# pliam1105/BoxFusion

Measured on AMD Instinct MI355X. Metric: RGB-D frames/sec (whole node) on 640x480 stream, higher is better.
Workload: dtype bf16; 1 GPU; configs[2]: synthetic 640x480 RGB-D, batch 8/step/GPU, gap=1, CuTR ViT-B RGB-D + CLIP ViT-H/14 x16 crops/frame + fusion; frames=440, global_batch=8, parallelism=dp1, inflight_batches_per_gpu=2, scene_objects=30, fused_boxes=83, global_boxes=30

## Files before the change

### boxfusion_amd/_lib.py

```python
from __future__ import annotations

import atexit
import ctypes
import threading
import weakref
import sys
import os

import numpy as np
import torch

HERE = os.path.dirname(os.path.abspath(__file__))
LIB_PATH = os.environ.get("BF_LIB_PATH") or os.path.join(HERE, "libboxfusion_hip.so")
_LIB = None

c_int, c_float, c_double, c_void_p, c_size_t = (ctypes.c_int, ctypes.c_float, ctypes.c_double,
                                                ctypes.c_void_p, ctypes.c_size_t)

BF_DEV_FUSION_LIST_OVERFLOW = 1
BF_DEV_HULL_OVERFLOW = 2
BF_DEV_VIEW_OVERFLOW = 4
BF_DEV_INDEX_RANGE = 8
BF_DEV_HULL_TRUNC = 16

# ... 539 lines not shown
    o_bs = sq * o.stride(0) if o_bs is None else o_bs
    if o_map is not None:
        _need(o_map, torch.int32, "o_map")
        if o_map.numel() < batch * sq:
            raise HipError(f"o_map has {o_map.numel()} rows < batch*sq = {batch * sq}")
    LL = ctypes.c_longlong
    _check(lib().bf_attention_bf16_ex(c_void_p(q.data_ptr()), c_void_p(k.data_ptr()),
                                      c_void_p(v.data_ptr()), c_void_p(o.data_ptr()), c_int(batch),
                                      c_int(heads), c_int(sq), c_int(sk), c_int(head_dim),
                                      c_int(q.stride(0)), c_int(k.stride(0)), c_int(v.stride(0)),
                                      c_int(o.stride(0)), LL(q_bs), LL(k_bs), LL(v_bs), LL(o_bs),
                                      c_float(scale), _ptr(o_map) if o_map is not None else None,
                                      c_int(variant or _knobs().get("attn_variant", 0)), _stream()),
           "bf_attention_bf16_ex")
    return o


def attention_fp8out(q, k, v, o, batch, heads, sq, sk, head_dim, scale, out_qscale, q_bs=None,
                     k_bs=None, v_bs=None, o_bs=None, variant=0):
    for x, n in ((q, "q"), (k, "k"), (v, "v")):
        _need(x, torch.bfloat16, n)
    _need(o, FP8, "o")
    q_bs = sq * q.stride(0) if q_bs is None else q_bs
    k_bs = sk * k.stride(0) if k_bs is None else k_bs
    v_bs = sk * v.stride(0) if v_bs is None else v_bs
    o_bs = sq * o.stride(0) if o_bs is None else o_bs
    LL = ctypes.c_longlong
    _check(lib().bf_attention_fp8out_ex(c_void_p(q.data_ptr()), c_void_p(k.data_ptr()), c_void_p(v.data_ptr()),
                                        c_void_p(o.data_ptr()), c_int(batch), c_int(heads), c_int(sq),
                                        c_int(sk), c_int(head_dim), c_int(q.stride(0)), c_int(k.stride(0)),
                                        c_int(v.stride(0)), c_int(o.stride(0)), LL(q_bs), LL(k_bs), LL(v_bs),
                                        LL(o_bs), c_float(scale), c_float(out_qscale),
                                        c_int(variant or _knobs().get("attn_variant", 0)), _stream()),
           "bf_attention_fp8out_ex")
    return o


def layernorm(x, weight, bias, eps, out=None, row_map=None, out_dtype=torch.bfloat16):
    _need(x, torch.float32, "x")
    M, C = x.shape
    if out is None:
        out = torch.empty((M, C), dtype=out_dtype, device=x.device)
    if out.dtype not in (torch.bfloat16, torch.float32) or x.stride(1) != 1 or out.stride(1) != 1:
        raise HipError("layernorm: f32 in, bf16 / f32 out, unit column stride")
    _check(lib().bf_layernorm_out(c_void_p(x.data_ptr()), c_int(x.stride(0)), _ptr(weight),
                                  _ptr(bias), c_float(eps), c_void_p(out.data_ptr()),
                                  c_int(out.stride(0)), c_int(int(out.dtype == torch.float32)),
                                  _ptr(row_map) if row_map is not None else None, c_int(M), c_int(C),
                                  _stream()), "bf_layernorm_out")
    return out



def attention_causal(q, k, v, o, batch, heads, s, head_dim, scale):
    for x, n in ((q, "q"), (k, "k"), (v, "v"), (o, "o")):
        _need(x, torch.bfloat16, n)
    LL = ctypes.c_longlong
    _check(lib().bf_attention_causal(c_void_p(q.data_ptr()), c_void_p(k.data_ptr()), c_void_p(v.data_ptr()),
                                     c_void_p(o.data_ptr()), c_int(batch), c_int(heads), c_int(s),
                                     c_int(head_dim), c_int(q.stride(0)), c_int(k.stride(0)),
                                     c_int(v.stride(0)), c_int(o.stride(0)), LL(s * q.stride(0)),
                                     LL(s * k.stride(0)), LL(s * v.stride(0)), LL(s * o.stride(0)),
                                     c_float(scale), _stream()), "bf_attention_causal")
    return o


def token_embed(ids, table, pos, out=None, status=None):
    _need(ids, torch.int32, "ids")
    _need(table, torch.float32, "table")
    _need(pos, torch.float32, "pos")
    N, S = ids.shape
    W = table.shape[1]
    if pos.shape[0] < S or pos.shape[1] != W:
        raise HipError(f"token_embed: positional table {tuple(pos.shape)} for S={S}, W={W}")
    if out is None:
        out = torch.empty((N * S, W), dtype=torch.float32, device=ids.device)
    _need(out, torch.float32, "out")
    own = status is None
    if own:
        status = torch.zeros(1, dtype=torch.int32, device=ids.device)
    _check(lib().bf_token_embed(_ptr(ids), c_int(N * S), _ptr(table), c_int(table.shape[0]), _ptr(pos),
                                c_int(S), c_int(W), _ptr(out), _ptr(status), _stream()), "bf_token_embed")
    if own and int(status.item()) & BF_DEV_INDEX_RANGE:
        raise HipError("bf_token_embed: a token id outside the vocabulary (BF_DEV_INDEX_RANGE)")
    return out


def text_pool(ids, x, out=None):
    _need(ids, torch.int32, "ids")
    _need(x, torch.float32, "x")
    N, S = ids.shape
    W = x.shape[1]
    if out is None:
        out = torch.empty((N, W), dtype=torch.float32, device=x.device)
    _need(out, torch.float32, "out")
    _check(lib().bf_text_pool(_ptr(ids), c_int(N), c_int(S), _ptr(x), c_int(W), _ptr(out), _stream()),
           "bf_text_pool")
    return out


def l2_normalize_rows(x, out=None):
    _need(x, torch.float32, "x")
    if out is None:
        out = torch.empty_like(x)
    _need(out, torch.float32, "out")
    _check(lib().bf_l2_normalize_rows(_ptr(x), c_int(x.shape[0]), c_int(x.shape[1]), _ptr(out), _stream()),
           "bf_l2_normalize_rows")
    return out


def ingest_rgbd(bgr, depth_u16, depth_scale, rot_k=0, rgb_out=None, depth_out=None, src_bgr=True):
    _need(bgr, torch.uint8, "bgr")
    if bgr.dim() == 3:
        bgr = bgr[None]
    F_, Hc, Wc, C = bgr.shape
    if C != 3:
# ... 722 lines not shown
```

### boxfusion_amd/csrc/bf_attn.hip

```cpp
#include "bf_common.h"

#include <type_traits>
#include <climits>
#include <algorithm>

typedef __bf16 bf16x8 __attribute__((ext_vector_type(8)));
typedef float f32x16 __attribute__((ext_vector_type(16)));
typedef unsigned short u16;

#define AT_THREADS 256
#define AT_QT 128
#define AT_KT 64

struct alignas(16) V128 {
    uint32_t x, y, z, w;
};
struct alignas(8) V64 {
    uint32_t x, y;
};

__device__ __forceinline__ u16 at_f2bf(float f) {
    __bf16 b = (__bf16)f;
    return *reinterpret_cast<u16*>(&b);
}

__device__ __forceinline__ long long attn_out_offset(const int32_t* __restrict__ o_map, int b, int q,
                                                     int sq, long long o_bs, int o_rs) {
    if (!o_map) return b * o_bs + (long long)q * o_rs;
    if (q >= sq) return -1;
    const int r = o_map[(long long)b * sq + q];
    return r < 0 ? -1 : (long long)r * o_rs;
}


typedef short s16x4 __attribute__((ext_vector_type(4)));


struct AttnBlk {
    int qb, h, b;
};
__device__ __forceinline__ AttnBlk attn_block(int remap) {
    const unsigned nx = gridDim.x, ny = gridDim.y, nz = gridDim.z;
    if (!remap) return AttnBlk{(int)blockIdx.x, (int)blockIdx.y, (int)blockIdx.z};
    const unsigned n = nx * ny * nz;
    const unsigned id = blockIdx.x + nx * (blockIdx.y + ny * blockIdx.z);
    const unsigned xcd = id % 8u, k = id / 8u, q = n / 8u, r = n % 8u;
    const unsigned lin = (xcd < r ? xcd * (q + 1) : r * (q + 1) + (xcd - r) * q) + k;
    return AttnBlk{(int)(lin % nx), (int)((lin / nx) % ny), (int)(lin / (nx * ny))};
}

__host__ __device__ constexpr int attn_vrow_bytes(int d) {
    int sb = 2 * d;
    while (sb % 256 != 64 && sb % 256 != 192) sb += 32;
    return sb;
}

#define AT2_THR 8.0f

template <int D, int DB, bool ONES>
__device__ __forceinline__ void attn2_softmax(f32x16 (&s)[2], bool sub1, bool mask, int k0, int sk,
                                              int fh, float c, float& m_run, float& l_run,
                                              f32x16 (&o)[DB], bf16x8 (&pf)[2][2], int kmax = INT_MAX) {
    if (mask) {
        const int klim = min(sk - 1, kmax);
#pragma unroll
        for (int sub = 0; sub < 2; ++sub)
#pragma unroll
            for (int e = 0; e < 16; ++e) {
                const int key = k0 + sub * 32 + (e & 3) + 8 * (e >> 2) + 4 * fh;
                s[sub][e] = (key <= klim) ? s[sub][e] : -INFINITY;
            }
    }
    float mt = s[0][0];
#pragma unroll
    for (int e = 1; e < 16; ++e) mt = fmaxf(mt, s[0][e]);
    if (sub1) {
#pragma unroll
        for (int e = 0; e < 16; ++e) mt = fmaxf(mt, s[1][e]);
    }
    mt = fmaxf(mt, __shfl_xor(mt, 32, 64)) * c;
    if (__any(mt > m_run + AT2_THR)) {
        const float m_new = fmaxf(m_run, mt);
        const float alpha = __builtin_amdgcn_exp2f(m_run - m_new);
        m_run = m_new;
        l_run *= alpha;
#pragma unroll
        for (int db = 0; db < DB; ++db)
#pragma unroll
            for (int e = 0; e < 16; ++e) o[db][e] *= alpha;
    }
    float ls = 0.f;
#pragma unroll
    for (int sub = 0; sub < 2; ++sub) {
        if (sub == 1 && !sub1) {
#pragma unroll
            for (int e = 0; e < 16; ++e) pf[1][e >> 3][e & 7] = (__bf16)0.0f;
            continue;
        }
#pragma unroll
        for (int e = 0; e < 16; ++e) {
            const float p = __builtin_amdgcn_exp2f(fmaf(s[sub][e], c, -m_run));
            if (!ONES) ls += p;
            pf[sub][e >> 3][e & 7] = (__bf16)p;
        }
    }
    if (!ONES) l_run += ls;
}

#ifndef ATTN_WPE64
#define ATTN_WPE64 3
#endif
#ifndef ATTN_WPE80
#define ATTN_WPE80 3
#endif
template <int D, int NW, bool F8O = false, bool CAUSAL = false, bool LSTQ = false>
__global__ void __launch_bounds__(NW * 64, (D == 64 && NW == 4) ? ATTN_WPE64 : (D == 80 && NW == 4 && !CAUSAL) ? ATTN_WPE80 : 1)
k_attn2(const u16* __restrict__ Q, const u16* __restrict__ K,
                                                      const u16* __restrict__ V, u16* __restrict__ O,
                                                      int sq, int sk, int q_rs, int k_rs, int v_rs,
                                                      int o_rs, long long q_bs, long long k_bs,
                                                      long long v_bs, long long o_bs, float scale_log2,
                                                      const int32_t* __restrict__ o_map, float oqs = 1.f) {
    constexpr int KS = D / 16;
    constexpr int DB = (D + 31) / 32;
    constexpr bool ONES = (D % 32) != 0;
    constexpr int KROW = D + 8;
    constexpr int VROW = attn_vrow_bytes(D) / 2;
    constexpr int KTILE = AT_KT * KROW;
    constexpr int VTILE = AT_KT * VROW;
    constexpr int CPR = D / 8;
    constexpr int CH = AT_KT * CPR;
    constexpr int NT = NW * 64;
    constexpr int NBUF = 2;
    __shared__ __attribute__((aligned(16))) u16 sK[NBUF * KTILE];
    __shared__ __attribute__((aligned(16))) u16 sV[NBUF * VTILE];
    constexpr bool LST = LSTQ && !CAUSAL && D % 16 == 0;
    constexpr int EB = F8O ? 1 : 2;
    constexpr int OROW = ((EB * D + 16) / 32) * 32 + 16;
    constexpr bool OWN = NW >= 8;
    static_assert(!LST || OWN || NW * 32 * OROW <= NBUF * KTILE * 2, "staged rows fit the K ring");
    __shared__ __attribute__((aligned(16))) unsigned char sO[LST && OWN ? NW * 32 * OROW : 16];

    const int t = threadIdx.x, lane = t & 63, wave = t >> 6;
    const AttnBlk blk = attn_block(1);
    const int h = blk.h, b = blk.b;
    const int fr = lane & 31, fh = lane >> 5;
    const int q = blk.qb * (NW * 32) + wave * 32 + fr;
    const bool idle = blk.qb * (NW * 32) + wave * 32 >= sq;
    const u16* Qb = Q + b * q_bs + h * D;
    const u16* Kb = K + b * k_bs + h * D;
    const u16* Vb = V + b * v_bs + h * D;

    bf16x8 qf[KS];
#pragma unroll
    for (int ks = 0; ks < KS; ++ks)
        qf[ks] = *reinterpret_cast<const bf16x8*>(Qb + (size_t)min(q, sq - 1) * q_rs + 16 * ks + 8 * fh);
    if (VROW > D)
        for (int i = t; i < NBUF * AT_KT * (VROW - D); i += NT) {
            const int r = i / (VROW - D), c = i % (VROW - D);
            sV[r * VROW + D + c] = (ONES && c == 0) ? (u16)0x3F80 : (u16)0;
        }

    static_assert(CH % 64 == 0 && NT % 64 == 0, "wave-uniform staging guard");
    constexpr int NTS = NT;
    const int ts = t;
    constexpr int NSO = (CH + NTS - 1) / NTS;
    typedef unsigned u32x4 __attribute__((ext_vector_type(4)));
    u32x4 stk[NSO], stv[NSO];
    int srow[NSO], scol[NSO];
#pragma unroll
    for (int i = 0; i < NSO; ++i) {
        const int c = min(ts + i * NTS, CH - 1);
        srow[i] = c / CPR;
        scol[i] = (c % CPR) * 8;
    }
    auto stage_load = [&](int k0_) {
#pragma unroll
        for (int i = 0; i < NSO; ++i) {
            const int key = min(k0_ + srow[i], sk - 1);
            stk[i] = *reinterpret_cast<const u32x4*>(Kb + (size_t)key * k_rs + scol[i]);
            stv[i] = *reinterpret_cast<const u32x4*>(Vb + (size_t)key * v_rs + scol[i]);
        }
    };
    auto stage_store = [&](int buf_) {
#pragma unroll
        for (int i = 0; i < NSO; ++i) {
            if (ts + i * NTS < CH) {
                *reinterpret_cast<u32x4*>(sK + buf_ * KTILE + srow[i] * KROW + scol[i]) = stk[i];
                *reinterpret_cast<u32x4*>(sV + buf_ * VTILE + srow[i] * VROW + scol[i]) = stv[i];
            }
        }
    };

    f32x16 o[DB];
#pragma unroll
    for (int db = 0; db < DB; ++db)
#pragma unroll
        for (int e = 0; e < 16; ++e) o[db][e] = 0.f;
    float m_run = -INFINITY, l_run = 0.f;
    const int g16 = (lane >> 4) & 1, q4 = (lane & 15) >> 2, p4 = lane & 3;
    const int ntiles = (sk + AT_KT - 1) / AT_KT;
    const int nfull = sk / AT_KT;

    auto qk = [&](int tile, f32x16 (&s)[2], bool maybe_tail) {
        const int k0 = tile * AT_KT;
        const u16* kt = sK + (tile % NBUF) * KTILE;
        const bool sub1 = !maybe_tail || (k0 + 32 < sk);
#pragma unroll
        for (int sub = 0; sub < 2; ++sub) {
            if (sub == 1 && !sub1) {
#pragma unroll
                for (int e = 0; e < 16; ++e) s[1][e] = -INFINITY;
                continue;
            }
#pragma unroll
            for (int ks = 0; ks < KS; ++ks) {
                bf16x8 kf = *reinterpret_cast<const bf16x8*>(kt + (sub * 32 + fr) * KROW + 16 * ks + 8 * fh);
                s[sub] = __builtin_amdgcn_mfma_f32_32x32x16_bf16(kf, qf[ks], ks == 0 ? f32x16{} : s[sub], 0, 0, 0);
            }
        }
    };
    auto sm_pv = [&](int tile, f32x16 (&s)[2], auto mask_tag) {
        constexpr bool MASK = decltype(mask_tag)::value;
        const int k0 = tile * AT_KT;
        const u16* kt = sK + (tile % NBUF) * KTILE;
        const u16* vt = sV + (tile % NBUF) * VTILE;
        const bool sub1 = !MASK || (k0 + 32 < sk);
        bf16x8 pf[2][2];
        attn2_softmax<D, DB, ONES>(s, sub1, MASK, k0, sk, fh, scale_log2, m_run, l_run, o, pf,
                                   CAUSAL ? q : INT_MAX);
#pragma unroll
        for (int db = 0; db < DB; ++db) {
            const int d0 = db * 32 + g16 * 16 + 4 * p4;
#pragma unroll
            for (int sub = 0; sub < 2; ++sub)
#pragma unroll
                for (int ss = 0; ss < 2; ++ss) {
                    if (MASK && sub == 1 && !sub1) continue;
                    const int kb = 32 * sub + 16 * ss + 4 * fh + q4;
                    typedef __attribute__((address_space(3))) s16x4* lds_s4;
                    const s16x4 lo = __builtin_amdgcn_ds_read_tr16_b64_v4i16((lds_s4)(vt + kb * VROW + d0));
                    const s16x4 hi = __builtin_amdgcn_ds_read_tr16_b64_v4i16((lds_s4)(vt + (kb + 8) * VROW + d0));
                    typedef short s16x8 __attribute__((ext_vector_type(8)));
                    const s16x8 lohi = __builtin_shufflevector(lo, hi, 0, 1, 2, 3, 4, 5, 6, 7);
                    o[db] = __builtin_amdgcn_mfma_f32_32x32x16_bf16(__builtin_bit_cast(bf16x8, lohi),
                                                                   pf[sub][ss], o[db], 0, 0, 0);
                }
        }
    };
    auto tile_body = [&](int tile, auto mask_tag) {
        f32x16 s[2];
        qk(tile, s, decltype(mask_tag)::value);
        sm_pv(tile, s, mask_tag);
    };

    stage_load(0);
    stage_store(0);
    __syncthreads();
    if constexpr (CAUSAL) {
        const int nt = min(ntiles, (min(blk.qb * (NW * 32) + NW * 32, sq) - 1) / AT_KT + 1);
        for (int tile = 0; tile < nt; ++tile) {
            const bool more = tile + 1 < nt;
            if (more) stage_load((tile + 1) * AT_KT);
            tile_body(tile, std::true_type{});
            if (more) stage_store((tile + 1) & 1);
            __syncthreads();
        }
    } else {
        for (int tile = 0; tile < nfull; ++tile) {
            const bool more = tile + 1 < ntiles;
            if (more) stage_load((tile + 1) * AT_KT);
            if (!idle) tile_body(tile, std::false_type{});
            if (more) stage_store((tile + 1) % NBUF);
            __syncthreads();
        }
        if (nfull < ntiles && !idle) tile_body(nfull, std::true_type{});
    }
    float l;
    if (ONES) {
        constexpr int rr = D % 32;
        constexpr int e_l = ((rr >> 3) << 2) | (rr & 3);
        constexpr int fh_l = (rr >> 2) & 1;
        const float mine = o[DB - 1][e_l];
        const float other = __shfl_xor(mine, 32, 64);
        l = (fh == fh_l) ? mine : other;
    } else {
        l = l_run + __shfl_xor(l_run, 32, 64);
    }
    if constexpr (LST) {
        const float inv = 1.0f / l;
        if constexpr (!OWN) __syncthreads();
        if (idle) return;
        unsigned char* wreg = (OWN ? sO : reinterpret_cast<unsigned char*>(sK)) + wave * 32 * OROW;
#pragma unroll
        for (int db = 0; db < DB; ++db)
#pragma unroll
            for (int g = 0; g < 4; ++g) {
                const int d0 = db * 32 + 8 * g + 4 * fh;
                if (d0 >= D) continue;
                if constexpr (F8O) {
                    const float sc = inv * oqs;
                    float a[4];
#pragma unroll
                    for (int i = 0; i < 4; ++i) a[i] = fminf(fmaxf(o[db][4 * g + i] * sc, -448.f), 448.f);
                    int pk = __builtin_amdgcn_cvt_pk_fp8_f32(a[0], a[1], 0, false);
                    pk = __builtin_amdgcn_cvt_pk_fp8_f32(a[2], a[3], pk, true);
                    *reinterpret_cast<int*>(wreg + fr * OROW + d0) = pk;
                } else {
                    V64 w;
                    w.x = (uint32_t)at_f2bf(o[db][4 * g + 0] * inv) | ((uint32_t)at_f2bf(o[db][4 * g + 1] * inv) << 16);
                    w.y = (uint32_t)at_f2bf(o[db][4 * g + 2] * inv) | ((uint32_t)at_f2bf(o[db][4 * g + 3] * inv) << 16);
                    *reinterpret_cast<V64*>(wreg + fr * OROW + 2 * d0) = w;
                }
            }
        constexpr int CPRO = EB * D / 16;
        unsigned char* Ob = reinterpret_cast<unsigned char*>(O);
#pragma unroll
        for (int j = 0; j < (32 * CPRO + 63) / 64; ++j) {
            const int c = lane + 64 * j;
            if (c >= 32 * CPRO) break;
            const int r = c / CPRO, col = c % CPRO;
            const int qr = q - fr + r;
            const V128 val = *reinterpret_cast<const V128*>(wreg + r * OROW + 16 * col);
            const long long off = attn_out_offset(o_map, b, qr, sq, o_bs, o_rs);
            if (qr < sq && off >= 0) *reinterpret_cast<V128*>(Ob + EB * (off + h * D) + 16 * col) = val;
        }
        return;
    }
    const long long o_off = attn_out_offset(o_map, b, q, sq, o_bs, o_rs);
    if (q < sq && o_off >= 0) {
        const float inv = 1.0f / l;
        if constexpr (F8O) {
            unsigned char* orow = reinterpret_cast<unsigned char*>(O) + o_off + h * D;
            const float sc = inv * oqs;
#pragma unroll
            for (int db = 0; db < DB; ++db)
#pragma unroll
                for (int g = 0; g < 4; ++g) {
                    const int d0 = db * 32 + 8 * g + 4 * fh;
                    if (d0 >= D) continue;
                    float a[4];
#pragma unroll
                    for (int i = 0; i < 4; ++i) a[i] = fminf(fmaxf(o[db][4 * g + i] * sc, -448.f), 448.f);
                    int pk = __builtin_amdgcn_cvt_pk_fp8_f32(a[0], a[1], 0, false);
                    pk = __builtin_amdgcn_cvt_pk_fp8_f32(a[2], a[3], pk, true);
                    *reinterpret_cast<int*>(orow + d0) = pk;
                }
        } else {
            u16* orow = O + o_off + h * D;
#pragma unroll
            for (int db = 0; db < DB; ++db)
#pragma unroll
                for (int g = 0; g < 4; ++g) {
                    const int d0 = db * 32 + 8 * g + 4 * fh;
                    if (d0 >= D) continue;
                    V64 w;
                    w.x = (uint32_t)at_f2bf(o[db][4 * g + 0] * inv) | ((uint32_t)at_f2bf(o[db][4 * g + 1] * inv) << 16);
                    w.y = (uint32_t)at_f2bf(o[db][4 * g + 2] * inv) | ((uint32_t)at_f2bf(o[db][4 * g + 3] * inv) << 16);
                    *reinterpret_cast<V64*>(orow + d0) = w;
                }
        }
    }
}
BF_API int bf_attention_bf16_ex(const void* q, const void* k, const void* v, void* o, int batch,
                                int heads, int sq, int sk, int head_dim, int q_rs, int k_rs,
                                int v_rs, int o_rs, long long q_bs, long long k_bs, long long v_bs,
                                long long o_bs, float scale, const int32_t* o_map, int variant,
                                void* stream) {
    const int av = variant == 0 ? 6 : variant;
    if (!q || !k || !v || !o || batch <= 0 || heads <= 0 || sq <= 0 || sk <= 0) return BF_ERR_ARG;
    if ((q_rs | k_rs | v_rs) % 8 != 0 || o_rs % 4 != 0) return BF_ERR_UNSUPPORTED;
    const float sl2 = scale * 1.4426950408889634f;
    const int nw_one = (sq + 31) / 32;
    const bool short_s = nw_one > 4 && nw_one <= 9;
    const bool lst = av != 27;
    const int mid = av == 28 ? 9 : av == 29 ? 4 : av == 30 ? 8
                  : (head_dim == 64 || head_dim == 80) ? 4 : 8;
    const bool four_all = av == 31;
    const int top = av == 28 ? 9 : (four_all || head_dim == 80) ? 4 : 9;
    const bool eight = short_s && nw_one <= 8 && mid == 8 && !four_all;
    const bool nine = short_s && !four_all && (nw_one <= 8 ? mid == 9 : top == 9);
    const bool wide8 = head_dim == 64 && sq > 448 && sq <= 512 && av != 33;
    const hipStream_t st = bf_stream(stream);
#define LAUNCH_2(DD, NWV, LS)                                                                     \
    hipLaunchKernelGGL((k_attn2<DD, NWV, false, false, LS>), dim3((sq + NWV * 32 - 1) / (NWV * 32), heads, batch), \
                       dim3(NWV * 64), 0, st, (const u16*)q, (const u16*)k, (const u16*)v, (u16*)o, sq, sk, \
                       q_rs, k_rs, v_rs, o_rs, q_bs, k_bs, v_bs, o_bs, sl2, o_map, 1.f)
#define LAUNCH_2D(DD)                                                                             \
    if (nw_one <= 2) { LAUNCH_2(DD, 2, false); }                                                  \
    else if (eight) { if (lst) { LAUNCH_2(DD, 8, true); } else { LAUNCH_2(DD, 8, false); } }      \
    else if (nine) { if (lst) { LAUNCH_2(DD, 9, true); } else { LAUNCH_2(DD, 9, false); } }       \
    else if (wide8) { if (lst) { LAUNCH_2(DD, 8, true); } else { LAUNCH_2(DD, 8, false); } }      \
    else { if (lst) { LAUNCH_2(DD, 4, true); } else { LAUNCH_2(DD, 4, false); } }
    switch (head_dim) {
        case 32: LAUNCH_2D(32); break;
        case 64: LAUNCH_2D(64); break;
        case 80: LAUNCH_2D(80); break;
        case 128: LAUNCH_2(128, 4, false); break;
        default: return BF_ERR_UNSUPPORTED;
    }
#undef LAUNCH_2D
#undef LAUNCH_2
    return bf_check_launch();
}

BF_API int bf_attention_bf16_omap(const void* q, const void* k, const void* v, void* o, int batch,
                                  int heads, int sq, int sk, int head_dim, int q_rs, int k_rs,
                                  int v_rs, int o_rs, long long q_bs, long long k_bs, long long v_bs,
                                  long long o_bs, float scale, const int32_t* o_map, void* stream) {
    return bf_attention_bf16_ex(q, k, v, o, batch, heads, sq, sk, head_dim, q_rs, k_rs, v_rs, o_rs, q_bs, k_bs,
                                v_bs, o_bs, scale, o_map, 0, stream);
}

BF_API int bf_attention_bf16(const void* q, const void* k, const void* v, void* o, int batch,
                             int heads, int sq, int sk, int head_dim, int q_rs, int k_rs, int v_rs,
                             int o_rs, long long q_bs, long long k_bs, long long v_bs,
                             long long o_bs, float scale, void* stream) {
    return bf_attention_bf16_omap(q, k, v, o, batch, heads, sq, sk, head_dim, q_rs, k_rs, v_rs, o_rs,
                                  q_bs, k_bs, v_bs, o_bs, scale, nullptr, stream);
}

BF_API int bf_attention_fp8out_ex(const void* q, const void* k, const void* v, void* o, int batch,
                                  int heads, int sq, int sk, int head_dim, int q_rs, int k_rs, int v_rs,
                                  int o_rs, long long q_bs, long long k_bs, long long v_bs, long long o_bs,
                                  float scale, float out_qscale, int variant, void* stream) {
    const int av = variant == 0 ? 6 : variant;
    if (!q || !k || !v || !o || batch <= 0 || heads <= 0 || sq <= 0 || sk <= 0 || !(out_qscale > 0.f))
        return BF_ERR_ARG;
    if ((q_rs | k_rs | v_rs) % 8 != 0 || o_rs % 4 != 0 || o_bs % 4 != 0) return BF_ERR_UNSUPPORTED;
    const float sl2 = scale * 1.4426950408889634f;
    const int nw_one = (sq + 31) / 32;
    const bool lst = av != 27;
    const hipStream_t st = bf_stream(stream);
#define LAUNCH_8(DD, NWV, LS)                                                                     \
    hipLaunchKernelGGL((k_attn2<DD, NWV, true, false, LS>), dim3((sq + NWV * 32 - 1) / (NWV * 32), heads, batch), \
                       dim3(NWV * 64), 0, st, (const u16*)q, (const u16*)k, (const u16*)v, (u16*)o, sq, sk, \
                       q_rs, k_rs, v_rs, o_rs, q_bs, k_bs, v_bs, o_bs, sl2, (const int32_t*)nullptr, out_qscale)
    const bool nine = nw_one > 4 && nw_one <= 9 && !(head_dim == 80 && nw_one == 9 && av != 28);
#define LAUNCH_8D(DD)                                                                             \
    if (nine) { if (lst) { LAUNCH_8(DD, 9, true); } else { LAUNCH_8(DD, 9, false); } }             \
    else { if (lst) { LAUNCH_8(DD, 4, true); } else { LAUNCH_8(DD, 4, false); } }
    switch (head_dim) {
        case 64: LAUNCH_8D(64); break;
        case 80: LAUNCH_8D(80); break;
        default: return BF_ERR_UNSUPPORTED;
    }
#undef LAUNCH_8D
#undef LAUNCH_8
    return bf_check_launch();
}

BF_API int bf_attention_fp8out(const void* q, const void* k, const void* v, void* o, int batch,
                               int heads, int sq, int sk, int head_dim, int q_rs, int k_rs, int v_rs,
                               int o_rs, long long q_bs, long long k_bs, long long v_bs, long long o_bs,
                               float scale, float out_qscale, void* stream) {
    return bf_attention_fp8out_ex(q, k, v, o, batch, heads, sq, sk, head_dim, q_rs, k_rs, v_rs, o_rs, q_bs, k_bs,
                                  v_bs, o_bs, scale, out_qscale, 0, stream);
}

BF_API int bf_attention_causal(const void* q, const void* k, const void* v, void* o, int batch, int heads,
                               int s, int head_dim, int q_rs, int k_rs, int v_rs, int o_rs, long long q_bs,
                               long long k_bs, long long v_bs, long long o_bs, float scale, void* stream) {
    if (!q || !k || !v || !o || batch <= 0 || heads <= 0 || s <= 0) return BF_ERR_ARG;
    if ((q_rs | k_rs | v_rs) % 8 != 0 || o_rs % 4 != 0) return BF_ERR_UNSUPPORTED;
    const float sl2 = scale * 1.4426950408889634f;
#define LAUNCH_C(DD)                                                                              \
    hipLaunchKernelGGL((k_attn2<DD, 4, false, true>), dim3((s + 127) / 128, heads, batch), dim3(256), \
                       0, bf_stream(stream), (const u16*)q, (const u16*)k, (const u16*)v, (u16*)o, s, s, \
                       q_rs, k_rs, v_rs, o_rs, q_bs, k_bs, v_bs, o_bs, sl2, (const int32_t*)nullptr, 1.f)
    switch (head_dim) {
        case 64: LAUNCH_C(64); break;
        case 80: LAUNCH_C(80); break;
        default: return BF_ERR_UNSUPPORTED;
    }
#undef LAUNCH_C
    return bf_check_launch();
}
```

### include/boxfusion_hip.h

```cpp
#ifndef BOXFUSION_HIP_H
#define BOXFUSION_HIP_H

#include <stdint.h>
#include <stddef.h>

#ifdef __cplusplus
extern "C" {
#endif

typedef enum {
    BF_OK = 0,
    BF_ERR_ARG = -1,
    BF_ERR_LAUNCH = -2,
    BF_ERR_CAPACITY = -3,
    BF_ERR_UNSUPPORTED = -4
} bf_status;

#define BF_DEV_OK 0
#define BF_DEV_FUSION_LIST_OVERFLOW 1
#define BF_DEV_HULL_OVERFLOW 2
#define BF_DEV_VIEW_OVERFLOW 4
#define BF_DEV_INDEX_RANGE 8
#define BF_DEV_HULL_TRUNC 16

// ... 212 lines not shown

int bf_gemm_f32(const float* A, int lda, const int* a_map, const float* W, int ldw,
                const float* bias, const float* resid, int ldr, float* C, int ldc,
                const int* c_map, int M, int N, int K, int act, void* stream);
int bf_ln_rows_f32(const float* x, int ldx, const float* gamma, const float* beta, float eps,
                   float* out, int ldo, const float* pos, int ldp, float* out2, int ldo2, int M,
                   int C, int gelu, void* stream);
int bf_groupnorm_cl_f32(const float* x, int ldx, int B, int P, int C, int G, const float* gamma,
                        const float* beta, float eps, float* out, int ldo, const float* pos,
                        int ldp, float* out2, int ldo2, void* stream);
int bf_s2d_f32(const float* x, int ldx, int B, int H, int W, int C, float* out, void* stream);
int bf_row_heads_f32(const float* x, int ldx, int in_fs, int in_off, int rows, int nq, int K,
                     const float* w, const float* b, int nout, const float* prop,
                     const float* params, float* out, int ldo, float* boxes, float clamp_w,
                     float clamp_h, float max_ratio, int mode, void* stream);
int bf_topk_rows_f32(const float* v, int ldv, int frames, int n, int k, int* idx, float* vals,
                     void* stream);
int bf_prop_select_f32(const float* boxes, int frames, int n, int k, const int* idx, float* ref,
                       const float* ex, const float* ey, const float* ew, const float* eh, int ed,
                       float max_e, float* qpos, int ldq, int qfs, int qoff, void* stream);
int bf_infer_select_f32(const float* logits, int frames, int nq, int nc, const float* boxes,
                        const float* b3info, const float* desc, int ld_desc, int desc_fs,
                        int desc_off, int C, const float* Kinv, const float* Tg,
                        const float* img_wh, int k, float* scores, long long* classes,
                        float* out_logits, float* out_boxes, float* out_proj, float* out_b3,
                        float* out_R, float* out_desc, void* stream);
int bf_ray_fourier_f32(float fx, float fy, float cx, float cy, int W, int H, int feat, int stride,
                       const float* scales, int nb, float* out, int ld, void* stream);

int bf_layernorm(const float* x, int ldx, const float* gamma, const float* beta, float eps,
                 void* out, int ldo, const int32_t* row_map, int M, int C, void* stream);
int bf_layernorm_out(const float* x, int ldx, const float* gamma, const float* beta, float eps,
                     void* out, int ldo, int out_f32, const int32_t* row_map, int M, int C,
                     void* stream);
int bf_layernorm_fp8(const float* x, int ldx, const float* gamma, const float* beta, float eps,
                     void* out, int ldo, float qscale, int M, int C, void* stream);

int bf_im2col_rgb8(const uint8_t* img, int B, int H, int W, int pad, int patch,
                   const float* mean3, const float* std3, void* out, int ldo, void* stream);
int bf_im2col_rgb8_chw(const uint8_t* img, int B, int H, int W, int chw, int pad, int patch,
                       const float* mean3, const float* std3, void* out, int ldo, void* stream);

int bf_im2col_f32(const float* x, int B, int H, int W, int pad, int patch, void* out, int ldo,
                  void* stream);

int bf_crop_resize_im2col(const uint8_t* img, int H, int W, const int32_t* boxes,
                          const int32_t* img_idx, int N, int size, int patch, const float* mean3,
                          const float* std3, void* out, int ldo, void* stream);


int bf_attention_causal(const void* q, const void* k, const void* v, void* o, int batch, int heads,
                        int s, int head_dim, int q_rs, int k_rs, int v_rs, int o_rs, long long q_bs,
                        long long k_bs, long long v_bs, long long o_bs, float scale, void* stream);

int bf_token_embed(const int32_t* ids, int n_tok, const float* table, int vocab, const float* pos,
                   int S, int W, float* out, int32_t* status, void* stream);

int bf_text_pool(const int32_t* ids, int N, int S, const float* x, int W, float* out, void* stream);

int bf_l2_normalize_rows(const float* x, int rows, int W, float* out, void* stream);


int bf_ingest_rgbd(const uint8_t* bgr, int Hc, int Wc, const uint16_t* depth, int Hd, int Wd, int F,
                   float depth_scale, int rot_k, int src_bgr, uint8_t* rgb_out, float* depth_out,
                   void* stream);

int bf_cv2_resize_u8(const uint8_t* src, int Hs, int Ws, int cn, int Hd, int Wd, int F, uint8_t* dst,
                     void* stream);

#define BF_PNG_BAD_SIGNATURE 1
#define BF_PNG_BAD_HEADER 2
#define BF_PNG_UNSUPPORTED 4
#define BF_PNG_BAD_CHUNK 8
#define BF_PNG_BAD_ZLIB 16
#define BF_PNG_BAD_ADLER 32
#define BF_PNG_BAD_FILTER 64
#define BF_PNG_SIZE 128
size_t bf_png_workspace_bytes(int F, int H, int W, long long total_file_bytes);
int bf_png_decode_u16(const uint8_t* files, const int64_t* offsets, int F, int H, int W,
                      long long total_file_bytes, long long max_file_bytes, uint16_t* out, void* work,
                      size_t work_bytes, int32_t* status, void* stream);
int bf_png_decode_depth(const uint8_t* files, const int64_t* offsets, int F, int H, int W,
                        long long total_file_bytes, long long max_file_bytes, float depth_scale,
                        float* depth_out, void* work, size_t work_bytes, int32_t* status, void* stream);

size_t bf_png_rgb_workspace_bytes(int F, int H, int W, long long total_file_bytes);
int bf_png_decode_rgb(const uint8_t* files, const int64_t* offsets, int F, int H, int W,
                      long long total_file_bytes, long long max_file_bytes, uint8_t* rgb,
                      void* work, size_t work_bytes, int32_t* status, void* stream);

#define BF_JPG_BAD_MARKER 1
#define BF_JPG_UNSUPPORTED 2
#define BF_JPG_SIZE 4
#define BF_JPG_BAD_DATA 8
size_t bf_jpeg_workspace_bytes(int F, int H, int W);
int bf_jpeg_decode_rgb(const uint8_t* files, const int64_t* offsets, int F, int H, int W, uint8_t* rgb,
                       void* work, size_t work_bytes, int32_t* status, void* stream);

int bf_cu_probe(int* out, int n_wg, int spin, void* stream);

#ifdef __cplusplus
}
#endif
#endif
```

Baseline: 146.5 frames/s.

## Trim attention kernel overheads: peel first tile, specialize tail, 32-bit addressing

Adds several compile-time trims to the flash-attention kernel, selected by an ATTN_TRIM mask. The first KV tile is peeled so the initial max is set directly without a rescale and the accumulators are not zeroed separately. The partial final tile gets a specialized softmax/PV path that only processes the valid key groups. Staging loads use precomputed 32-bit byte offsets and wave-uniform indices, and padding stores are vectorized. The previous code path is kept as a 'PF' variant, used when row strides are too wide for 32-bit offsets or when variant 34 is requested. A causal _ex entry point with a variant argument is added. The main gain is in ALU and address arithmetic in attention, at the cost of more template instantiations and code size.

```diff
diff --git a/boxfusion_amd/_lib.py b/boxfusion_amd/_lib.py
--- a/boxfusion_amd/_lib.py
+++ b/boxfusion_amd/_lib.py
@@ -615,16 +615,16 @@
 
 
 
-def attention_causal(q, k, v, o, batch, heads, s, head_dim, scale):
+def attention_causal(q, k, v, o, batch, heads, s, head_dim, scale, variant=0):
     for x, n in ((q, "q"), (k, "k"), (v, "v"), (o, "o")):
         _need(x, torch.bfloat16, n)
     LL = ctypes.c_longlong
-    _check(lib().bf_attention_causal(c_void_p(q.data_ptr()), c_void_p(k.data_ptr()), c_void_p(v.data_ptr()),
-                                     c_void_p(o.data_ptr()), c_int(batch), c_int(heads), c_int(s),
-                                     c_int(head_dim), c_int(q.stride(0)), c_int(k.stride(0)),
-                                     c_int(v.stride(0)), c_int(o.stride(0)), LL(s * q.stride(0)),
-                                     LL(s * k.stride(0)), LL(s * v.stride(0)), LL(s * o.stride(0)),
-                                     c_float(scale), _stream()), "bf_attention_causal")
+    _check(lib().bf_attention_causal_ex(c_void_p(q.data_ptr()), c_void_p(k.data_ptr()), c_void_p(v.data_ptr()),
+                                        c_void_p(o.data_ptr()), c_int(batch), c_int(heads), c_int(s),
+                                        c_int(head_dim), c_int(q.stride(0)), c_int(k.stride(0)),
+                                        c_int(v.stride(0)), c_int(o.stride(0)), LL(s * q.stride(0)),
+                                        LL(s * k.stride(0)), LL(s * v.stride(0)), LL(s * o.stride(0)),
+                                        c_float(scale), c_int(variant), _stream()), "bf_attention_causal_ex")
     return o
 
 
diff --git a/boxfusion_amd/csrc/bf_attn.hip b/boxfusion_amd/csrc/bf_attn.hip
--- a/boxfusion_amd/csrc/bf_attn.hip
+++ b/boxfusion_amd/csrc/bf_attn.hip
@@ -57,7 +57,7 @@
 
 #define AT2_THR 8.0f
 
-template <int D, int DB, bool ONES>
+template <int D, int DB, bool ONES, bool FIRST = false>
 __device__ __forceinline__ void attn2_softmax(f32x16 (&s)[2], bool sub1, bool mask, int k0, int sk,
                                               int fh, float c, float& m_run, float& l_run,
                                               f32x16 (&o)[DB], bf16x8 (&pf)[2][2], int kmax = INT_MAX) {
@@ -78,6 +78,50 @@
 #pragma unroll
         for (int e = 0; e < 16; ++e) mt = fmaxf(mt, s[1][e]);
     }
+    mt = fmaxf(mt, __shfl_xor(mt, 32, 64)) * c;
+    if constexpr (FIRST) {
+        m_run = mt;
+    } else if (__any(mt > m_run + AT2_THR)) {
+        const float m_new = fmaxf(m_run, mt);
+        const float alpha = __builtin_amdgcn_exp2f(m_run - m_new);
+        m_run = m_new;
+        l_run *= alpha;
+#pragma unroll
+        for (int db = 0; db < DB; ++db)
+#pragma unroll
+            for (int e = 0; e < 16; ++e) o[db][e] *= alpha;
+    }
+    float ls = 0.f;
+#pragma unroll
+    for (int sub = 0; sub < 2; ++sub) {
+        if (sub == 1 && !sub1) {
+#pragma unroll
+            for (int e = 0; e < 16; ++e) pf[1][e >> 3][e & 7] = (__bf16)0.0f;
+            continue;
+        }
+#pragma unroll
+        for (int e = 0; e < 16; ++e) {
+            const float p = __builtin_amdgcn_exp2f(fmaf(s[sub][e], c, -m_run));
+            if (!ONES) ls += p;
+            pf[sub][e >> 3][e & 7] = (__bf16)p;
+        }
+    }
+    if (!ONES) l_run += ls;
+}
+
+template <int DB, bool ONES, int NG>
+__device__ __forceinline__ void attn2_softmax_tail(f32x16 (&s)[2], int lim, float c, float& m_run,
+                                                   float& l_run, f32x16 (&o)[DB], bf16x8 (&pf)[2][2]) {
+    constexpr int GL = NG - 1;
+#pragma unroll
+    for (int e8 = 0; e8 < 8; ++e8) {
+        const int e = 8 * (GL & 1) + e8;
+        const int koff = 32 * (GL >> 1) + (e & 3) + 8 * (e >> 2);
+        s[GL >> 1][e] = (koff < lim) ? s[GL >> 1][e] : -INFINITY;
+    }
+    float mt = s[0][0];
+#pragma unroll
+    for (int i = 1; i < 8 * NG; ++i) mt = fmaxf(mt, s[i >> 4][i & 15]);
     mt = fmaxf(mt, __shfl_xor(mt, 32, 64)) * c;
     if (__any(mt > m_run + AT2_THR)) {
         const float m_new = fmaxf(m_run, mt);
@@ -91,18 +135,10 @@
     }
     float ls = 0.f;
 #pragma unroll
-    for (int sub = 0; sub < 2; ++sub) {
-        if (sub == 1 && !sub1) {
-#pragma unroll
-            for (int e = 0; e < 16; ++e) pf[1][e >> 3][e & 7] = (__bf16)0.0f;
-            continue;
-        }
-#pragma unroll
-        for (int e = 0; e < 16; ++e) {
-            const float p = __builtin_amdgcn_exp2f(fmaf(s[sub][e], c, -m_run));
-            if (!ONES) ls += p;
-            pf[sub][e >> 3][e & 7] = (__bf16)p;
-        }
+    for (int i = 0; i < 8 * NG; ++i) {
+        const float p = __builtin_amdgcn_exp2f(fmaf(s[i >> 4][i & 15], c, -m_run));
+        if (!ONES) ls += p;
+        pf[i >> 4][(i >> 3) & 1][i & 7] = (__bf16)p;
     }
     if (!ONES) l_run += ls;
 }
@@ -113,7 +149,10 @@
 #ifndef ATTN_WPE80
 #define ATTN_WPE80 3
 #endif
-template <int D, int NW, bool F8O = false, bool CAUSAL = false, bool LSTQ = false>
+#ifndef ATTN_TRIM
+#define ATTN_TRIM 15
+#endif
+template <int D, int NW, bool F8O = false, bool CAUSAL = false, bool LSTQ = false, bool PF = false>
 __global__ void __launch_bounds__(NW * 64, (D == 64 && NW == 4) ? ATTN_WPE64 : (D == 80 && NW == 4 && !CAUSAL) ? ATTN_WPE80 : 1)
 k_attn2(const u16* __restrict__ Q, const u16* __restrict__ K,
                                                       const u16* __restrict__ V, u16* __restrict__ O,
@@ -141,45 +180,97 @@
     static_assert(!LST || OWN || NW * 32 * OROW <= NBUF * KTILE * 2, "staged rows fit the K ring");
     __shared__ __attribute__((aligned(16))) unsigned char sO[LST && OWN ? NW * 32 * OROW : 16];
 
-    const int t = threadIdx.x, lane = t & 63, wave = t >> 6;
+    constexpr bool T_TAIL = !PF && (ATTN_TRIM & 1) && !(D == 64 && NW == 8), T_PEEL = !PF && (ATTN_TRIM & 2);
+    constexpr bool T_ADDR = !PF && (ATTN_TRIM & 4), T_EPI = !PF && (ATTN_TRIM & 8);
+    const int t = threadIdx.x, lane = t & 63;
+    const int wave = !(T_ADDR || T_EPI) ? t >> 6 : __builtin_amdgcn_readfirstlane(t >> 6);
     const AttnBlk blk = attn_block(1);
     const int h = blk.h, b = blk.b;
     const int fr = lane & 31, fh = lane >> 5;
-    const int q = blk.qb * (NW * 32) + wave * 32 + fr;
-    const bool idle = blk.qb * (NW * 32) + wave * 32 >= sq;
+    const int q0w = blk.qb * (NW * 32) + wave * 32;
+    const int q = q0w + fr;
+    const bool idle = q0w >= sq;
     const u16* Qb = Q + b * q_bs + h * D;
     const u16* Kb = K + b * k_bs + h * D;
     const u16* Vb = V + b * v_bs + h * D;
+    typedef unsigned u32x4 __attribute__((ext_vector_type(4)));
+    const int ntiles = (sk + AT_KT - 1) / AT_KT;
+    const int nfull = sk / AT_KT;
 
     bf16x8 qf[KS];
-#pragma unroll
-    for (int ks = 0; ks < KS; ++ks)
-        qf[ks] = *reinterpret_cast<const bf16x8*>(Qb + (size_t)min(q, sq - 1) * q_rs + 16 * ks + 8 * fh);
-    if (VROW > D)
-        for (int i = t; i < NBUF * AT_KT * (VROW - D); i += NT) {
-            const int r = i / (VROW - D), c = i % (VROW - D);
-            sV[r * VROW + D + c] = (ONES && c == 0) ? (u16)0x3F80 : (u16)0;
-        }
+    if constexpr (!T_ADDR) {
+#pragma unroll
+        for (int ks = 0; ks < KS; ++ks)
+            qf[ks] = *reinterpret_cast<const bf16x8*>(Qb + (size_t)min(q, sq - 1) * q_rs + 16 * ks + 8 * fh);
+        if (VROW > D)
+            for (int i = t; i < NBUF * AT_KT * (VROW - D); i += NT) {
+                const int r = i / (VROW - D), c = i % (VROW - D);
+                sV[r * VROW + D + c] = (ONES && c == 0) ? (u16)0x3F80 : (u16)0;
+            }
+    } else {
+        const unsigned char* qw = reinterpret_cast<const unsigned char*>(Qb + (size_t)min(q0w, sq - 1) * q_rs);
+        const unsigned qo = 2u * ((unsigned)min(fr, max(sq - 1 - q0w, 0)) * (unsigned)q_rs + 8u * fh);
+#pragma unroll
+        for (int ks = 0; ks < KS; ++ks) {
+            if (idle) qf[ks] = bf16x8{};
+            else qf[ks] = *reinterpret_cast<const bf16x8*>(qw + qo + 32 * ks);
+        }
+        constexpr int PC = (VROW - D) / 8;
+        static_assert((VROW - D) % 8 == 0 && (PC & (PC - 1)) == 0, "V padding in 16-byte chunks");
+        if constexpr (PC > 0) {
+#pragma unroll
+            for (int i0 = 0; i0 < NBUF * AT_KT * PC; i0 += NT) {
+                const int i = i0 + t;
+                if (i0 + NT <= NBUF * AT_KT * PC || i < NBUF * AT_KT * PC) {
+                    const int r = i / PC, c = i % PC;
+                    const u32x4 pad = {(ONES && c == 0) ? 0x3F80u : 0u, 0u, 0u, 0u};
+                    *reinterpret_cast<u32x4*>(sV + r * VROW + D + 8 * c) = pad;
+                }
+            }
+        }
+    }
 
     static_assert(CH % 64 == 0 && NT % 64 == 0, "wave-uniform staging guard");
     constexpr int NTS = NT;
     const int ts = t;
     constexpr int NSO = (CH + NTS - 1) / NTS;
-    typedef unsigned u32x4 __attribute__((ext_vector_type(4)));
     u32x4 stk[NSO], stv[NSO];
     int srow[NSO], scol[NSO];
+    unsigned kofs[NSO], vofs[NSO];
 #pragma unroll
     for (int i = 0; i < NSO; ++i) {
         const int c = min(ts + i * NTS, CH - 1);
         srow[i] = c / CPR;
         scol[i] = (c % CPR) * 8;
+        kofs[i] = 2u * ((unsigned)srow[i] * (unsigned)k_rs + scol[i]);
+        vofs[i] = 2u * ((unsigned)srow[i] * (unsigned)v_rs + scol[i]);
     }
     auto stage_load = [&](int k0_) {
-#pragma unroll
-        for (int i = 0; i < NSO; ++i) {
-            const int key = min(k0_ + srow[i], sk - 1);
-            stk[i] = *reinterpret_cast<const u32x4*>(Kb + (size_t)key * k_rs + scol[i]);
-            stv[i] = *reinterpret_cast<const u32x4*>(Vb + (size_t)key * v_rs + scol[i]);
+        if constexpr (!T_ADDR) {
+#pragma unroll
+            for (int i = 0; i < NSO; ++i) {
+                const int key = min(k0_ + srow[i], sk - 1);
+                stk[i] = *reinterpret_cast<const u32x4*>(Kb + (size_t)key * k_rs + scol[i]);
+                stv[i] = *reinterpret_cast<const u32x4*>(Vb + (size_t)key * v_rs + scol[i]);
+            }
+        } else {
+            const unsigned char* kt_ = reinterpret_cast<const unsigned char*>(Kb + (size_t)k0_ * k_rs);
+            const unsigned char* vt_ = reinterpret_cast<const unsigned char*>(Vb + (size_t)k0_ * v_rs);
+            if (k0_ + AT_KT <= sk) {
+#pragma unroll
+                for (int i = 0; i < NSO; ++i) {
+                    stk[i] = *reinterpret_cast<const u32x4*>(kt_ + kofs[i]);
+                    stv[i] = *reinterpret_cast<const u32x4*>(vt_ + vofs[i]);
+                }
+            } else {
+                const int rmax = sk - 1 - k0_;
+#pragma unroll
+                for (int i = 0; i < NSO; ++i) {
+                    const unsigned r = (unsigned)min(srow[i], rmax);
+                    stk[i] = *reinterpret_cast<const u32x4*>(kt_ + 2u * (r * (unsigned)k_rs + scol[i]));
+                    stv[i] = *reinterpret_cast<const u32x4*>(vt_ + 2u * (r * (unsigned)v_rs + scol[i]));
+                }
+            }
         }
     };
     auto stage_store = [&](int buf_) {
@@ -192,15 +283,17 @@
         }
     };
 
+    constexpr bool PEEL = T_PEEL && !CAUSAL;
     f32x16 o[DB];
-#pragma unroll
-    for (int db = 0; db < DB; ++db)
-#pragma unroll
-        for (int e = 0; e < 16; ++e) o[db][e] = 0.f;
+    auto zero_o = [&]() {
+#pragma unroll
+        for (int db = 0; db < DB; ++db)
+#pragma unroll
+            for (int e = 0; e < 16; ++e) o[db][e] = 0.f;
+    };
+    if (!PEEL) zero_o();
     float m_run = -INFINITY, l_run = 0.f;
     const int g16 = (lane >> 4) & 1, q4 = (lane & 15) >> 2, p4 = lane & 3;
-    const int ntiles = (sk + AT_KT - 1) / AT_KT;
-    const int nfull = sk / AT_KT;
 
     auto qk = [&](int tile, f32x16 (&s)[2], bool maybe_tail) {
         const int k0 = tile * AT_KT;
@@ -220,38 +313,63 @@
             }
         }
     };
-    auto sm_pv = [&](int tile, f32x16 (&s)[2], auto mask_tag) {
+    auto pv = [&](const u16* vt, int db, int sub, int ss, const bf16x8& p, bool zc) {
+        const int d0 = db * 32 + g16 * 16 + 4 * p4;
+        const int kb = 32 * sub + 16 * ss + 4 * fh + q4;
+        typedef __attribute__((address_space(3))) s16x4* lds_s4;
+        const s16x4 lo = __builtin_amdgcn_ds_read_tr16_b64_v4i16((lds_s4)(vt + kb * VROW + d0));
+        const s16x4 hi = __builtin_amdgcn_ds_read_tr16_b64_v4i16((lds_s4)(vt + (kb + 8) * VROW + d0));
+        typedef short s16x8 __attribute__((ext_vector_type(8)));
+        const s16x8 lohi = __builtin_shufflevector(lo, hi, 0, 1, 2, 3, 4, 5, 6, 7);
+        o[db] = __builtin_amdgcn_mfma_f32_32x32x16_bf16(__builtin_bit_cast(bf16x8, lohi), p,
+                                                       zc ? f32x16{} : o[db], 0, 0, 0);
+    };
+    auto sm_pv = [&](int tile, f32x16 (&s)[2], auto mask_tag, auto first_tag) {
         constexpr bool MASK = decltype(mask_tag)::value;
+        constexpr bool FIRST = decltype(first_tag)::value;
         const int k0 = tile * AT_KT;
-        const u16* kt = sK + (tile % NBUF) * KTILE;
         const u16* vt = sV + (tile % NBUF) * VTILE;
         const bool sub1 = !MASK || (k0 + 32 < sk);
         bf16x8 pf[2][2];
-        attn2_softmax<D, DB, ONES>(s, sub1, MASK, k0, sk, fh, scale_log2, m_run, l_run, o, pf,
-                                   CAUSAL ? q : INT_MAX);
-#pragma unroll
-        for (int db = 0; db < DB; ++db) {
-            const int d0 = db * 32 + g16 * 16 + 4 * p4;
+        attn2_softmax<D, DB, ONES, FIRST>(s, sub1, MASK, k0, sk, fh, scale_log2, m_run, l_run, o, pf,
+                                          CAUSAL ? q : INT_MAX);
+#pragma unroll
+        for (int db = 0; db < DB; ++db)
 #pragma unroll
             for (int sub = 0; sub < 2; ++sub)
 #pragma unroll
                 for (int ss = 0; ss < 2; ++ss) {
                     if (MASK && sub == 1 && !sub1) continue;
-                    const int kb = 32 * sub + 16 * ss + 4 * fh + q4;
-                    typedef __attribute__((address_space(3))) s16x4* lds_s4;
-                    const s16x4 lo = __builtin_amdgcn_ds_read_tr16_b64_v4i16((lds_s4)(vt + kb * VROW + d0));
-                    const s16x4 hi = __builtin_amdgcn_ds_read_tr16_b64_v4i16((lds_s4)(vt + (kb + 8) * VROW + d0));
-                    typedef short s16x8 __attribute__((ext_vector_type(8)));
-                    const s16x8 lohi = __builtin_shufflevector(lo, hi, 0, 1, 2, 3, 4, 5, 6, 7);
-                    o[db] = __builtin_amdgcn_mfma_f32_32x32x16_bf16(__builtin_bit_cast(bf16x8, lohi),
-                                                                   pf[sub][ss], o[db], 0, 0, 0);
-                }
-        }
-    };
-    auto tile_body = [&](int tile, auto mask_tag) {
+                    pv(vt, db, sub, ss, pf[sub][ss], FIRST && sub == 0 && ss == 0);
+                }
+    };
+    auto tile_body = [&](int tile, auto mask_tag, auto first_tag) {
         f32x16 s[2];
         qk(tile, s, decltype(mask_tag)::value);
-        sm_pv(tile, s, mask_tag);
+        sm_pv(tile, s, mask_tag, first_tag);
+    };
+    auto tail_body = [&](auto ng_tag) {
+        constexpr int NG = decltype(ng_tag)::value;
+        const int k0 = nfull * AT_KT;
+        const u16* kt = sK + (nfull % NBUF) * KTILE;
+        const u16* vt = sV + (nfull % NBUF) * VTILE;
+        f32x16 s[2];
+#pragma unroll
+        for (int sub = 0; sub < (NG + 1) / 2; ++sub)
+#pragma unroll
+            for (int ks = 0; ks < KS; ++ks) {
+                bf16x8 kf = *reinterpret_cast<const bf16x8*>(kt + (sub * 32 + fr) * KROW + 16 * ks + 8 * fh);
+                s[sub] = __builtin_amdgcn_mfma_f32_32x32x16_bf16(kf, qf[ks], ks == 0 ? f32x16{} : s[sub], 0, 0, 0);
+            }
+        bf16x8 pf[2][2];
+        __builtin_amdgcn_sched_barrier(0);
+        attn2_softmax_tail<DB, ONES, NG>(s, sk - k0 - 4 * fh, scale_log2, m_run, l_run, o, pf);
+#pragma unroll
+        for (int db = 0; db < DB; ++db) {
+            __builtin_amdgcn_sched_barrier(0);
+#pragma unroll
+            for (int g = 0; g < NG; ++g) pv(vt, db, g >> 1, g & 1, pf[g >> 1][g & 1], false);
+        }
     };
 
     stage_load(0);
@@ -262,19 +380,42 @@
         for (int tile = 0; tile < nt; ++tile) {
             const bool more = tile + 1 < nt;
             if (more) stage_load((tile + 1) * AT_KT);
-            tile_body(tile, std::true_type{});
+            tile_body(tile, std::true_type{}, std::false_type{});
             if (more) stage_store((tile + 1) & 1);
             __syncthreads();
         }
     } else {
-        for (int tile = 0; tile < nfull; ++tile) {
+        if constexpr (PEEL) {
+            if (nfull > 0) {
+                const bool more = 1 < ntiles;
+                if (more) stage_load(AT_KT);
+                if (!idle) tile_body(0, std::false_type{}, std::true_type{});
+                else zero_o();
+                if (more) stage_store(1);
+                __syncthreads();
+            } else {
+                zero_o();
+            }
+        }
+        for (int tile = PEEL ? 1 : 0; tile < nfull; ++tile) {
             const bool more = tile + 1 < ntiles;
             if (more) stage_load((tile + 1) * AT_KT);
-            if (!idle) tile_body(tile, std::false_type{});
+            if (!idle) tile_body(tile, std::false_type{}, std::false_type{});
             if (more) stage_store((tile + 1) % NBUF);
             __syncthreads();
         }
-        if (nfull < ntiles && !idle) tile_body(nfull, std::true_type{});
+        if (nfull < ntiles && !idle) {
+            if constexpr (!T_TAIL) {
+                tile_body(nfull, std::true_type{}, std::false_type{});
+            } else {
+                switch ((sk - nfull * AT_KT + 15) >> 4) {
+                    case 1: tail_body(std::integral_constant<int, 1>{}); break;
+                    case 2: tail_body(std::integral_constant<int, 2>{}); break;
+                    case 3: tail_body(std::integral_constant<int, 3>{}); break;
+                    default: tail_body(std::integral_constant<int, 4>{}); break;
+                }
+            }
+        }
     }
     float l;
     if (ONES) {
@@ -315,6 +456,19 @@
             }
         constexpr int CPRO = EB * D / 16;
         unsigned char* Ob = reinterpret_cast<unsigned char*>(O);
+        if (T_EPI && !o_map) {
+            unsigned char* ow = Ob + EB * (b * o_bs + (long long)q0w * o_rs + h * D);
+            const int nrow = sq - q0w;
+#pragma unroll
+            for (int j = 0; j < (32 * CPRO + 63) / 64; ++j) {
+                const int c = lane + 64 * j;
+                if (c >= 32 * CPRO) break;
+                const int r = c / CPRO, col = c % CPRO;
+                const V128 val = *reinterpret_cast<const V128*>(wreg + r * OROW + 16 * col);
+                if (r < nrow) *reinterpret_cast<V128*>(ow + (unsigned)(EB * r * o_rs + 16 * col)) = val;
+            }
+            return;
+        }
 #pragma unroll
         for (int j = 0; j < (32 * CPRO + 63) / 64; ++j) {
             const int c = lane + 64 * j;
@@ -361,6 +515,11 @@
                 }
         }
     }
+}
+static bool attn_wide_rows(int q_rs, int k_rs, int v_rs, int o_rs) {
+    const int lim = 1 << 23;
+    return q_rs >= lim || k_rs >= lim || v_rs >= lim || o_rs >= lim || q_rs < 0 || k_rs < 0 || v_rs < 0 ||
+           o_rs < 0;
 }
 BF_API int bf_attention_bf16_ex(const void* q, const void* k, const void* v, void* o, int batch,
                                 int heads, int sq, int sk, int head_dim, int q_rs, int k_rs,
@@ -374,6 +533,7 @@
     const int nw_one = (sq + 31) / 32;
     const bool short_s = nw_one > 4 && nw_one <= 9;
     const bool lst = av != 27;
+    const bool pform = av == 34 || attn_wide_rows(q_rs, k_rs, v_rs, o_rs);
     const int mid = av == 28 ? 9 : av == 29 ? 4 : av == 30 ? 8
                   : (head_dim == 64 || head_dim == 80) ? 4 : 8;
     const bool four_all = av == 31;
@@ -383,9 +543,14 @@
     const bool wide8 = head_dim == 64 && sq > 448 && sq <= 512 && av != 33;
     const hipStream_t st = bf_stream(stream);
 #define LAUNCH_2(DD, NWV, LS)                                                                     \
-    hipLaunchKernelGGL((k_attn2<DD, NWV, false, false, LS>), dim3((sq + NWV * 32 - 1) / (NWV * 32), heads, batch), \
-                       dim3(NWV * 64), 0, st, (const u16*)q, (const u16*)k, (const u16*)v, (u16*)o, sq, sk, \
-                       q_rs, k_rs, v_rs, o_rs, q_bs, k_bs, v_bs, o_bs, sl2, o_map, 1.f)
+    if (pform)                                                                                    \
+        hipLaunchKernelGGL((k_attn2<DD, NWV, false, false, LS, true>), dim3((sq + NWV * 32 - 1) / (NWV * 32), heads, batch), \
+                           dim3(NWV * 64), 0, st, (const u16*)q, (const u16*)k, (const u16*)v, (u16*)o, sq, sk, \
+                           q_rs, k_rs, v_rs, o_rs, q_bs, k_bs, v_bs, o_bs, sl2, o_map, 1.f);      \
+    else                                                                                          \
+        hipLaunchKernelGGL((k_attn2<DD, NWV, false, false, LS, false>), dim3((sq + NWV * 32 - 1) / (NWV * 32), heads, batch), \
+                           dim3(NWV * 64), 0, st, (const u16*)q, (const u16*)k, (const u16*)v, (u16*)o, sq, sk, \
+                           q_rs, k_rs, v_rs, o_rs, q_bs, k_bs, v_bs, o_bs, sl2, o_map, 1.f)
 #define LAUNCH_2D(DD)                                                                             \
     if (nw_one <= 2) { LAUNCH_2(DD, 2, false); }                                                  \
     else if (eight) { if (lst) { LAUNCH_2(DD, 8, true); } else { LAUNCH_2(DD, 8, false); } }      \
@@ -396,7 +561,7 @@
         case 32: LAUNCH_2D(32); break;
         case 64: LAUNCH_2D(64); break;
         case 80: LAUNCH_2D(80); break;
-        case 128: LAUNCH_2(128, 4, false); break;
+        case 128: { LAUNCH_2(128, 4, false); } break;
         default: return BF_ERR_UNSUPPORTED;
     }
 #undef LAUNCH_2D
@@ -431,11 +596,17 @@
     const float sl2 = scale * 1.4426950408889634f;
     const int nw_one = (sq + 31) / 32;
     const bool lst = av != 27;
+    const bool pform = av == 34 || attn_wide_rows(q_rs, k_rs, v_rs, o_rs);
     const hipStream_t st = bf_stream(stream);
 #define LAUNCH_8(DD, NWV, LS)                                                                     \
-    hipLaunchKernelGGL((k_attn2<DD, NWV, true, false, LS>), dim3((sq + NWV * 32 - 1) / (NWV * 32), heads, batch), \
-                       dim3(NWV * 64), 0, st, (const u16*)q, (const u16*)k, (const u16*)v, (u16*)o, sq, sk, \
-                       q_rs, k_rs, v_rs, o_rs, q_bs, k_bs, v_bs, o_bs, sl2, (const int32_t*)nullptr, out_qscale)
+    if (pform)                                                                                    \
+        hipLaunchKernelGGL((k_attn2<DD, NWV, true, false, LS, true>), dim3((sq + NWV * 32 - 1) / (NWV * 32), heads, batch), \
+                           dim3(NWV * 64), 0, st, (const u16*)q, (const u16*)k, (const u16*)v, (u16*)o, sq, sk, \
+                           q_rs, k_rs, v_rs, o_rs, q_bs, k_bs, v_bs, o_bs, sl2, (const int32_t*)nullptr, out_qscale); \
+    else                                                                                          \
+        hipLaunchKernelGGL((k_attn2<DD, NWV, true, false, LS, false>), dim3((sq + NWV * 32 - 1) / (NWV * 32), heads, batch), \
+                           dim3(NWV * 64), 0, st, (const u16*)q, (const u16*)k, (const u16*)v, (u16*)o, sq, sk, \
+                           q_rs, k_rs, v_rs, o_rs, q_bs, k_bs, v_bs, o_bs, sl2, (const int32_t*)nullptr, out_qscale)
     const bool nine = nw_one > 4 && nw_one <= 9 && !(head_dim == 80 && nw_one == 9 && av != 28);
 #define LAUNCH_8D(DD)                                                                             \
     if (nine) { if (lst) { LAUNCH_8(DD, 9, true); } else { LAUNCH_8(DD, 9, false); } }             \
@@ -458,21 +629,30 @@
                                   v_bs, o_bs, scale, out_qscale, 0, stream);
 }
 
+BF_API int bf_attention_causal_ex(const void* q, const void* k, const void* v, void* o, int batch, int heads,
+                                  int s, int head_dim, int q_rs, int k_rs, int v_rs, int o_rs, long long q_bs,
+                                  long long k_bs, long long v_bs, long long o_bs, float scale, int variant,
+                                  void* stream) {
+    if (!q || !k || !v || !o || batch <= 0 || heads <= 0 || s <= 0) return BF_ERR_ARG;
+    if ((q_rs | k_rs | v_rs) % 8 != 0 || o_rs % 4 != 0) return BF_ERR_UNSUPPORTED;
+    const float sl2 = scale * 1.4426950408889634f;
+    const bool pform = variant == 34 || attn_wide_rows(q_rs, k_rs, v_rs, o_rs);
+#define LAUNCH_C(DD, PFV)                                                                         \
+    hipLaunchKernelGGL((k_attn2<DD, 4, false, true, false, PFV>), dim3((s + 127) / 128, heads, batch), dim3(256), \
+                       0, bf_stream(stream), (const u16*)q, (const u16*)k, (const u16*)v, (u16*)o, s, s, \
+                       q_rs, k_rs, v_rs, o_rs, q_bs, k_bs, v_bs, o_bs, sl2, (const int32_t*)nullptr, 1.f)
+    switch (head_dim) {
+        case 64: if (pform) { LAUNCH_C(64, true); } else { LAUNCH_C(64, false); } break;
+        case 80: if (pform) { LAUNCH_C(80, true); } else { LAUNCH_C(80, false); } break;
+        default: return BF_ERR_UNSUPPORTED;
+    }
+#undef LAUNCH_C
+    return bf_check_launch();
+}
+
 BF_API int bf_attention_causal(const void* q, const void* k, const void* v, void* o, int batch, int heads,
                                int s, int head_dim, int q_rs, int k_rs, int v_rs, int o_rs, long long q_bs,
                                long long k_bs, long long v_bs, long long o_bs, float scale, void* stream) {
-    if (!q || !k || !v || !o || batch <= 0 || heads <= 0 || s <= 0) return BF_ERR_ARG;
-    if ((q_rs | k_rs | v_rs) % 8 != 0 || o_rs % 4 != 0) return BF_ERR_UNSUPPORTED;
-    const float sl2 = scale * 1.4426950408889634f;
-#define LAUNCH_C(DD)                                                                              \
-    hipLaunchKernelGGL((k_attn2<DD, 4, false, true>), dim3((s + 127) / 128, heads, batch), dim3(256), \
-                       0, bf_stream(stream), (const u16*)q, (const u16*)k, (const u16*)v, (u16*)o, s, s, \
-                       q_rs, k_rs, v_rs, o_rs, q_bs, k_bs, v_bs, o_bs, sl2, (const int32_t*)nullptr, 1.f)
-    switch (head_dim) {
-        case 64: LAUNCH_C(64); break;
-        case 80: LAUNCH_C(80); break;
-        default: return BF_ERR_UNSUPPORTED;
-    }
-#undef LAUNCH_C
-    return bf_check_launch();
-}
+    return bf_attention_causal_ex(q, k, v, o, batch, heads, s, head_dim, q_rs, k_rs, v_rs, o_rs, q_bs, k_bs,
+                                  v_bs, o_bs, scale, 0, stream);
+}
diff --git a/include/boxfusion_hip.h b/include/boxfusion_hip.h
--- a/include/boxfusion_hip.h
+++ b/include/boxfusion_hip.h
@@ -288,6 +288,10 @@
 int bf_attention_causal(const void* q, const void* k, const void* v, void* o, int batch, int heads,
                         int s, int head_dim, int q_rs, int k_rs, int v_rs, int o_rs, long long q_bs,
                         long long k_bs, long long v_bs, long long o_bs, float scale, void* stream);
+int bf_attention_causal_ex(const void* q, const void* k, const void* v, void* o, int batch, int heads,
+                           int s, int head_dim, int q_rs, int k_rs, int v_rs, int o_rs, long long q_bs,
+                           long long k_bs, long long v_bs, long long o_bs, float scale, int variant,
+                           void* stream);
 
 int bf_token_embed(const int32_t* ids, int n_tok, const float* table, int vocab, const float* pos,
                    int S, int W, float* out, int32_t* status, void* stream);
```

Result: no change. 147.1 frames/s, median of 6 (+0.4%).
